# vnminin/phylomap

Measured on NVIDIA B200. Metric: sampled branch-site histories/sec (4-state, 10k-tip tree), higher is better.
Workload: dtype f32

## Files before the change

### phylomap_b200/csrc/pm_host.cu

```cuda
#include <cuda_runtime.h>

#include <algorithm>
#include <chrono>
#include <cmath>
#include <cstdarg>
#include <cstdio>
#include <cstdlib>
#include <cstring>
#include <map>
#include <memory>
#include <mutex>
#include <string>
#include <type_traits>
#include <vector>

#include "../../include/phylomap_b200.h"
#include "pm_launch.cuh"
#include "pm_setup_kernels.cuh"
#include "pm_loglik.cuh"
#include "pm_exp.cuh"
#include "pm_nccl.hpp"
#include "pm_rates.hpp"
#include "pm_tree.hpp"

// ... 859 lines not shown
    const int ntr = ntrees;
    if (n < 2 || n > PM_NMAX) fail(PM_ERR_ARG, "number of states must be in 2..%d", PM_NMAX);
    if (!V.multi && ntr != 1) fail(PM_ERR_ARG, "this sampler takes exactly one tree");
    if (ntr < 1) fail(PM_ERR_ARG, "no trees");
    if (N_total < 0) fail(PM_ERR_ARG, "N must be non-negative");
    if (V.hidden && (n < 4 || (n & 1))) fail(PM_ERR_ARG, "hidden-rate samplers need an even number of states >= 4");
    if (V.two_state && n != 2) fail(PM_ERR_ARG, "this sampler is 2-state only");
    if (V.dic && n > PM_DIC_NMAX) fail(PM_ERR_ARG, "the DIC samplers support at most %d states", PM_DIC_NMAX);
    const int need_prior = V.two_state ? 4 : variant == PM_V_KSMT ? 8 : V.hidden ? 6 : 0;
    if (nprior < need_prior || (need_prior && !prior_)) fail(PM_ERR_ARG, "prior needs %d values", need_prior);
    if (need_prior) prior.assign(prior_, prior_ + nprior);
    pid.assign(pid_, pid_ + n);
    exact = opt.mode == PM_MODE_DETERMINISTIC;
    if (exact && opt.precision != PM_F64) fail(PM_ERR_ARG, "deterministic mode computes in FP64");
    if (exact && V.exp) fail(PM_ERR_ARG, "the direct sampler (maketreelistEXP) runs in production arithmetic only");
    if (opt.rng == PM_RNG_TABLE && (!opt.tab_off || !opt.tab_u)) fail(PM_ERR_ARG, "replay table missing");
    if (opt.rng == PM_RNG_TABLE && !exact) fail(PM_ERR_ARG, "the replay table feeds the deterministic mode only");
    if (opt.rng == PM_RNG_TABLE && (opt.site_offset != 0 || opt.allreduce || opt.nccl_world > 1)) fail(PM_ERR_ARG, "replay runs are single-process");
    if (opt.allreduce && !opt.cuda_stream)
      fail(PM_ERR_ARG, "an allreduce callback needs pm_options.cuda_stream: the collective must be ordered on the stream the chain launches on");
    if (opt.allreduce && opt.nccl_world > 1) fail(PM_ERR_ARG, "give either an allreduce callback or an NCCL clique, not both");
    if (opt.nccl_world > 1 && (!opt.nccl_id || opt.nccl_rank < 0 || opt.nccl_rank >= opt.nccl_world)) fail(PM_ERR_ARG, "bad NCCL clique (nccl_id / nccl_rank / nccl_world)");
    NS = (n == 2) ? 2 : (n == 4) ? 4 : 0;
    W = n + n * n + 1 + (V.dic ? 1 : 0);
    WR = W + 1;
    ncols = ncols_of(variant, n);

    if (!(Omega > 0)) fail(PM_ERR_ARG, "Omega must be positive");
    std::vector<pm::host::Schedule> schedules(ntr);
    for (int ti = 0; ti < ntr; ti++) {
      const pm_tree& x = tr[ti];
      if (x.n_tips != tr[0].n_tips || x.n_edges != tr[0].n_edges) fail(PM_ERR_ARG, "all trees must have the same number of tips");
      if (x.n_sites < 1 || x.n_sites != tr[0].n_sites) fail(PM_ERR_ARG, "n_sites must be >= 1 and equal across trees");
      if (x.n_sites >= (1LL << 31)) fail(PM_ERR_ARG, "at most 2^31 - 1 sites per process");
      if (!x.edge || !x.nen || !x.nodelist || !x.maps_off || !x.maps_len) fail(PM_ERR_ARG, "tree %d: missing field", ti);
      if (!x.states && !x.states_u8) fail(PM_ERR_ARG, "tree %d: states missing", ti);
      try {
        pm::host::build_schedule(x.n_tips, x.n_edges, x.edge, x.nen, x.nodelist, x.root, V.redraw_tips, schedules[ti]);
      } catch (const std::string& msg) { fail(PM_ERR_ARG, "tree %d: %s", ti, msg.c_str()); }
      if (x.maps_off[0] != 0) fail(PM_ERR_ARG, "tree %d: maps_off[0] must be 0", ti);
      for (int e = 0; e < x.n_edges; e++) {
        const long long a = x.maps_off[e], b = x.maps_off[e + 1];
        if (b <= a) fail(PM_ERR_ARG, "tree %d: branch %d has no segments", ti, e + 1);
        if (b - a > 65535) fail(PM_ERR_ARG, "tree %d: branch %d has more than 65535 segments", ti, e + 1);
        for (long long p = a; p < b; p++) {
          if (!(x.maps_len[p] >= 0)) fail(PM_ERR_ARG, "tree %d: negative or NA segment length", ti);
          if (x.maps_state && (x.maps_state[p] < 1 || x.maps_state[p] > n)) fail(PM_ERR_ARG, "tree %d: mapnames out of range", ti);
        }
      }
    }
    return schedules;
  }

  int open_device() {
    int ndev = 0;
    if (cudaGetDeviceCount(&ndev) != cudaSuccess || ndev <= 0) fail(PM_ERR_CUDA, "no CUDA device (there is no CPU fallback)");
    if (opt.device < 0 || opt.device >= ndev) fail(PM_ERR_CUDA, "device %d not present", opt.device);
    CK(cudaSetDevice(opt.device));
    int major = 0, minor = 0, sms = 0;
    CK(cudaDeviceGetAttribute(&major, cudaDevAttrComputeCapabilityMajor, opt.device));
    CK(cudaDeviceGetAttribute(&minor, cudaDevAttrComputeCapabilityMinor, opt.device));
    CK(cudaDeviceGetAttribute(&sms, cudaDevAttrMultiProcessorCount, opt.device));
    if (major != 10) fail(PM_ERR_CUDA, "device %d is sm_%d%d; this library is built for sm_100a only", opt.device, major, minor);
    if (opt.cuda_stream) stream = (cudaStream_t)opt.cuda_stream;
    else { CK(cudaStreamCreateWithFlags(&stream, cudaStreamNonBlocking)); own_stream = true; }
    return sms;
  }

  std::unique_ptr<TreeDev<Real>> create_tree(const pm_tree& x, int ti, pm::host::Schedule&& sch, int sms, cudaStream_t aux,
                                             double& tmax, PhaseTrace& trace) {
    std::unique_ptr<TreeDev<Real>> tp(new TreeDev<Real>());
    TreeDev<Real>& t = *tp;
    t.sch = std::move(sch);
    t.S = x.n_sites;
    t.TS = (t.S + 15) / 16 * 16;
    const int E = x.n_edges, T = x.n_tips;
    const long long S = t.S;
    const bool no_paths = V.exp || V.llonly;
    upload_tips(t, x, aux);
    std::vector<long long> moff(x.maps_off, x.maps_off + E + 1);
    std::vector<Real> elen(E);
    for (int e = 0; e < E; e++) {
      double tot = 0;
      for (long long p = moff[e]; p < moff[e + 1]; p++) tot = tot + x.maps_len[p];
      elen[e] = (Real)tot;
      tmax = std::max(tmax, tot);
    }
    std::vector<double> mlen(x.maps_len, x.maps_len + moff[E]);

    const size_t small_smem = with_ns([&](auto ns) { return pm::Sweep<Real, decltype(ns)::value, false>::small_smem(T); });
    const SmallChoice small = choose_small_kernel(!exact && (NS == 2 || NS == 4) && !no_paths && opt.rng != PM_RNG_TABLE, elen,
                                                  Omega, T, S, sms, small_smem, sw);
    t.small_ok = small.ok;
    t.small_two = small.two;
    const bool pooled_ok = !t.small_ok && !exact && !no_paths && sw.rec_pool;
    RecordPlan rp = plan_records(pooled_ok ? 5 : 0, elen, moff, S, Omega, exact, no_paths, opt.path_capacity);
    if (!rp.fits) rp = plan_records(0, elen, moff, S, Omega, exact, no_paths, opt.path_capacity);
    t.rec_shift = rp.rec_shift;
    t.rec_groups = (S + (1LL << t.rec_shift) - 1) >> t.rec_shift;
    t.chunk = rp.chunk;
    t.paths_grid = dim3((unsigned)rp.gx, (unsigned)rp.ny, 1);
    t.nblocks = rp.gx * rp.ny;
    t.small_chunks = (int)rp.ny;
    t.cap_off_h = std::move(rp.cap_off);
    trace.mark("record capacities");

    plan_partials_slots(t, sms);
    upload(t.up_entries, t.sch.up_entries, stream);
    upload(t.up_off, t.sch.up_off, stream);
    if (!exact && (NS == 2 || NS == 4)) {
      CladeCode cc = encode_clade_schedule(t.sch, S, t.TS, (long long)t.pl_sites * n * (long long)sizeof(Real), V.redraw_tips);
      upload(t.cl_entries, cc.e16, stream);
      upload(t.cl_warp_off, cc.cs.warp_off, stream);
      upload(t.cl_top_entries, cc.top, stream);
      upload(t.cl_top_off, cc.cs.top_off, stream);
      upload(t.cd_entries, cc.d16, stream);
      upload(t.cd_warp_off, cc.cs.down_warp_off, stream);
      upload(t.cd_top, cc.cs.down_top, stream);
      upload(t.cd_top_off, cc.cs.down_top_off, stream);
      upload(t.cd_tips, cc.tips, stream);
      t.P.n_cl_top_levels = (int)cc.cs.top_off.size() - 1;
      t.P.n_cd_top_levels = (int)cc.cs.down_top_off.size() - 1;
      t.P.n_cd_tips = (int)cc.tips.size() / 2;
      if (t.small_ok) {
        const SmallOrder so = small_draw_order(t.sch, cc.cs, elen);
        upload(t.small_down, so.down, stream);
        upload(t.small_border, so.border, stream);
        t.small_order_n = (int)so.border.size();
      }
    }
    upload(t.down_entries, t.sch.down_entries, stream);
    upload(t.down_off, t.sch.down_off, stream);
    upload(t.e_parent, t.sch.e_parent, stream);
    upload(t.e_child, t.sch.e_child, stream);
    upload(t.e_len, elen, stream);
    if (V.dic || V.exp) {
      std::vector<double> eld(E);
      for (int e = 0; e < E; e++) eld[e] = x.edge_length ? x.edge_length[e] : (double)elen[e];
      if (x.edge_length) for (int e = 0; e < E; e++) if (!(eld[e] >= 0)) fail(PM_ERR_ARG, "tree %d: negative or NA edge.length", ti);
      upload(t.e_len_d, eld, stream);
      t.TP.alloc((size_t)E * n * n * sizeof(Real));
      t.ll_partial.alloc((size_t)((S + 31) / 32) * sizeof(double));
    }
    trace.mark("clade schedules + uploads");
    alloc_path_state(t, moff, mlen, elen, sms);
    trace.mark("device buffers");
    return tp;
  }

  void upload_tips(TreeDev<Real>& t, const pm_tree& x, cudaStream_t aux) {
    const int T = x.n_tips;
    t.tipcode.alloc((size_t)T * t.TS);
    CK(cudaMemsetAsync(t.tipcode.p, 0, t.tipcode.bytes, aux));
    t.node_state.alloc((size_t)(2 * T - 1) * t.S);
    CK(cudaMemsetAsync(t.node_state.p, 0, t.node_state.bytes, aux));
    const size_t esz = x.states_u8 ? 1 : 4;
    long long rows_per = std::max<long long>(32, (256LL << 20) / ((long long)T * (long long)esz));
    rows_per = std::min<long long>(rows_per, std::min<long long>(t.S, 32LL * 65535));
    t.tip_stage.alloc((size_t)rows_per * T * esz);
    for (long long s0 = 0; s0 < t.S; s0 += rows_per) {
      const int ns = (int)std::min<long long>(rows_per, t.S - s0);
      const void* src = x.states_u8 ? (const void*)(x.states_u8 + s0 * T) : (const void*)(x.states + s0 * T);
      CK(cudaMemcpyAsync(t.tip_stage.p, src, (size_t)ns * T * esz, cudaMemcpyHostToDevice, aux));
      dim3 g((T + 31) / 32, (ns + 31) / 32), b(32, 8);
      if (x.states_u8)
        pm::k_init_tips<uint8_t><<<g, b, 0, aux>>>(t.tip_stage.template as<uint8_t>(), ns, s0, t.S, t.TS, T, n, V.parity_tips,
                                                     t.tipcode.template as<uint8_t>(), t.node_state.template as<uint8_t>(), err_flag.as<unsigned>());
      else
        pm::k_init_tips<int32_t><<<g, b, 0, aux>>>(t.tip_stage.template as<int32_t>(), ns, s0, t.S, t.TS, T, n, V.parity_tips,
                                                     t.tipcode.template as<uint8_t>(), t.node_state.template as<uint8_t>(), err_flag.as<unsigned>());
    }
    CK(cudaGetLastError());
  }

  void plan_partials_slots(TreeDev<Real>& t, int sms) {
    t.pl_slots = 0;
    t.pl_sites = t.S;
    if (exact || !(NS == 2 || NS == 4) || V.dic || V.exp || V.llonly || !sw.fused) return;
    const size_t smem_lo = ((size_t)n * n + 3 * n) * sizeof(Real);
    const int per_sm = with_ns([&](auto ns) { return pm::Sweep<Real, decltype(ns)::value, false>::fused_blocks_per_sm(smem_lo); });
    if (per_sm < 1) fail(PM_ERR_CUDA, "cudaOccupancyMaxActiveBlocksPerMultiprocessor failed for the fused prune + node-draw kernel");
    t.slots_per_sm = per_sm;
    t.pl_slots = sm_id_range(opt.device, sms) * per_sm;
    t.pl_sites = 32LL * t.pl_slots;
    if (t.pl_sites >= ((t.S + 31) / 32) * 32) {
      t.pl_slots = (int)((t.S + 31) / 32); t.pl_sites = 32LL * t.pl_slots; t.slots_per_sm = 0;
    } else {
      t.slot_busy.alloc((size_t)t.pl_slots * sizeof(int));
      CK(cudaMemsetAsync(t.slot_busy.p, 0, t.slot_busy.bytes, stream));
    }
  }

  void alloc_path_state(TreeDev<Real>& t, const std::vector<long long>& moff, const std::vector<double>& mlen,
                        const std::vector<Real>& elen, int sms) {
    const int E = t.sch.E, T = t.sch.T;
    const long long S = t.S, R = t.cap_off_h.back();
    const bool no_paths = V.exp || V.llonly;
    upload(t.maps_off, moff, stream);
    upload(t.maps_len, mlen, stream);
    upload(t.cap_off, t.cap_off_h, stream);
    if (!no_paths) t.meta.alloc((size_t)E * S * sizeof(uint32_t));
    t.PL.alloc((size_t)(T - 1) * t.pl_sites * n * sizeof(Real));
    for (int b = 0; b < 2 && !no_paths; b++) {
      t.rec_len[b].alloc((size_t)R * t.rec_groups * sizeof(Real));
      t.rec_st[b].alloc((size_t)R * t.rec_groups);
    }
    if (!exact && !no_paths) {
      const long long Wl = (S + 31) / 32;
      t.hard_ballot.alloc((size_t)E * Wl * sizeof(uint32_t));
      const WorkItems w = build_work_items(elen, Omega, S);
      t.wk_total = w.off.back();
      upload(t.wk_hint, w.hint, stream);
      upload(t.wk_off, w.off, stream);
      upload(t.wk_g, w.g, stream);
      t.wk_item.alloc((size_t)std::max<long long>(t.wk_total, 1) * sizeof(unsigned long long));
      pm::k_build_items<<<(unsigned)((t.wk_total + 255) / 256), 256, 0, stream>>>(t.wk_off.template as<long long>(), t.wk_g.template as<int>(), E, Wl,
                                                                                 t.wk_total, t.wk_item.template as<unsigned long long>());
      t.rec_cursor.alloc((size_t)t.small_chunks * t.rec_groups * sizeof(int));
      t.shape.alloc((size_t)E * S * sizeof(uint16_t));
      t.hard_blocks = (int)std::max<long long>(1, std::min<long long>(sms * 4LL, (t.wk_total + 3) / 4));
    }
    t.dw_rows = t.nblocks + 3 * t.hard_blocks;
    t.dw_partial.alloc((size_t)t.dw_rows * n * sizeof(double));
    CK(cudaMemsetAsync(t.dw_partial.p, 0, t.dw_partial.bytes, stream));
    dev_bytes += t.tipcode.bytes + t.node_state.bytes + t.meta.bytes + t.PL.bytes + 2 * (t.rec_len[0].bytes + t.rec_st[0].bytes) +
                 t.dw_partial.bytes + t.hard_ballot.bytes + t.rec_cursor.bytes + t.shape.bytes + t.wk_item.bytes;
  }

  void alloc_model_and_host_buffers(double tmax) {
    jcap = opt.power_capacity > 0 ? opt.power_capacity : 64;
    if (V.exp) jcap = 302;
    else if (opt.power_capacity <= 0) {
      const double lam = Omega * tmax;
      const double want = lam + 10 * std::sqrt(lam) + 24;
      jcap = (int)std::min(16384.0, std::max(64.0, want));
    }
    if (jcap < 2) jcap = 2;
    model.alloc((model_stride() + (size_t)jcap * n * n) * sizeof(Real));
    CK(cudaMallocHost((void**)&model_h, (model_stride() + (size_t)jcap * n * n) * sizeof(Real)));
    memset(model_h, 0, (model_stride() + (size_t)jcap * n * n) * sizeof(Real));
    CK(cudaMallocHost((void**)&rows_h, (size_t)ntrees * WR * sizeof(double)));
    if (cudaHostGetDevicePointer((void**)&rows_h_dev, rows_h, 0) != cudaSuccess) { rows_h_dev = nullptr; (void)cudaGetLastError(); }
    if (opt.nccl_world > 1) nccl = clique(opt.nccl_id, opt.nccl_world, opt.nccl_rank);
    CK(cudaMallocHost((void**)&err_h, sizeof(unsigned)));
    CK(cudaMallocHost((void**)&ctl_h, 2 * sizeof(uint32_t)));
    ctl.alloc(2 * sizeof(uint32_t));
    phase_ns.alloc(2 * sizeof(unsigned long long));
    CK(cudaMemsetAsync(phase_ns.p, 0, phase_ns.bytes, stream));
    if (V.dic) { CK(cudaMallocHost((void**)&q_h, (size_t)n * n * sizeof(double))); q_dev.alloc((size_t)n * n * sizeof(double)); }
    cnt.alloc((size_t)n * n * sizeof(unsigned long long));
    root_out.alloc(sizeof(int));
    CK(cudaMemsetAsync(cnt.p, 0, cnt.bytes, stream));
    CK(cudaMemsetAsync(root_out.p, 0, root_out.bytes, stream));
  }

  int replay_slots_per_iter() const { return (2 * trees[0]->sch.T - 1) + 2 * trees[0]->sch.E; }
  void upload_replay_table() {
    const long long nslots = (long long)ntrees * trees[0]->S * N_total * replay_slots_per_iter();
    std::vector<long long> off(nslots + 1);
    for (long long i = 0; i <= nslots; i++) off[i] = opt.tab_off[i];
    std::vector<double> u(opt.tab_u, opt.tab_u + off[nslots]);
    upload(tab_off, off, stream);
    upload(tab_u, u, stream);
    if (opt.host_tab) replay.reset(new pm::host::ReplaySource(opt.host_tab, opt.host_tab_n));
  }

  void fill_params(TreeDev<Real>& t, int ti) {
    pm::ChainParams<Real>& P = t.P;
    const int T = t.sch.T, E = t.sch.E, spi = replay_slots_per_iter();
    P.n = n; P.T = T; P.E = E; P.S = t.S;
    P.cap_off = t.cap_off.template as<int>();
    P.hard_ballot = t.hard_ballot.template as<uint32_t>(); P.W = (int)((t.S + 31) / 32);
    P.wk_off = t.wk_off.template as<long long>(); P.wk_g = t.wk_g.template as<int>(); P.wk_total = t.wk_total;
    P.wk_hint = t.wk_hint.template as<int>(); P.wk_item = t.wk_item.template as<unsigned long long>();
    P.rec_cursor = t.rec_cursor.template as<int>(); P.chunk = t.chunk; P.easy_blocks = t.nblocks;
    P.shape = t.shape.template as<uint16_t>();
    P.model = model.as<Real>(); P.ppow = model.as<Real>() + model_stride(); P.jcap = jcap;
    P.up_entries = t.up_entries.template as<int>(); P.up_off = t.up_off.template as<int>();
    P.n_up_levels = (int)t.sch.up_off.size() - 1;
    P.cl_entries = t.cl_entries.template as<int>(); P.cl_warp_off = t.cl_warp_off.template as<int>();
    P.cl_top_entries = t.cl_top_entries.template as<int>(); P.cl_top_off = t.cl_top_off.template as<int>();
    P.cd_top = t.cd_top.template as<int>(); P.cd_top_off = t.cd_top_off.template as<int>();
    P.cd_entries = t.cd_entries.template as<int>(); P.cd_warp_off = t.cd_warp_off.template as<int>();
    P.cd_tips = t.cd_tips.template as<long long>();
    P.down_entries = t.down_entries.template as<int>(); P.down_off = t.down_off.template as<int>();
    P.n_down_levels = (int)t.sch.down_off.size() - 1;
    P.e_parent = t.e_parent.template as<int>(); P.e_child = t.e_child.template as<int>();
    P.e_len = t.e_len.template as<Real>();
    P.maps_off = t.maps_off.template as<long long>(); P.maps_len = t.maps_len.template as<double>();
    P.root = t.sch.root;
    P.tipcode = t.tipcode.template as<uint8_t>(); P.TS = t.TS; P.node_state = t.node_state.template as<uint8_t>();
    P.meta = t.meta.template as<uint32_t>(); P.PL = t.PL.template as<Real>();
    P.tile_base = 0; P.pl_S = t.pl_sites; P.rec_shift = t.rec_shift; P.rec_groups = t.rec_groups; P.ctl = nullptr;
    for (int b = 0; b < 2; b++) { P.rec_len[b] = t.rec_len[b].template as<Real>(); P.rec_st[b] = t.rec_st[b].template as<uint8_t>(); }
    P.normalize = V.normalize || !exact; P.full_counts = V.full_counts; P.parity_tips = V.parity_tips;
    P.dw_partial = t.dw_partial.template as<double>(); P.cnt = cnt.as<unsigned long long>();
    P.root_out = root_out.as<int>(); P.err_flag = err_flag.as<unsigned>();
    const uint64_t key = opt.seed + (uint64_t)ti * 0x9E3779B97F4A7C15ull;
    P.rng.k0 = (uint32_t)key; P.rng.k1 = (uint32_t)(key >> 32);
    for (int r = 0; r < 10; r++) { P.rng.rk[2 * r] = P.rng.k0 + (uint32_t)r * 0x9E3779B9u; P.rng.rk[2 * r + 1] = P.rng.k1 + (uint32_t)r * 0xBB67AE85u; }
    P.rng.site0 = (uint32_t)opt.site_offset;
    P.rng.tab_off = opt.rng == PM_RNG_TABLE ? (const int64_t*)tab_off.p : nullptr;
    P.rng.tab_u = opt.rng == PM_RNG_TABLE ? tab_u.as<double>() : nullptr;
    P.rng.tab_site_stride = (int64_t)N_total * spi;
    P.rng.tab_base = (int64_t)ti * t.S * N_total * spi;
    P.rng.slots_per_iter = spi; P.rng.n_nodes = 2 * T - 1;
  }

  void reduce_over_ranks(double* buf, int count) {
    if (nccl) {
      auto& api = pm::host::NcclApi::get();
      const int rc = api.AllReduce(buf, buf, (size_t)count, pm::host::NcclApi::kDouble, pm::host::NcclApi::kSum, nccl, stream);
      if (rc != 0) fail(PM_ERR_CUDA, "ncclAllReduce failed: %s", api.error(rc).c_str());
    } else if (opt.allreduce) {
      if (opt.allreduce(opt.allreduce_ctx, buf, count) != 0) fail(PM_ERR_CUDA, "allreduce callback failed");
    }
  }
  void check_row_errors(const double* rows_host, int nrows) {
    bool any = false;
    for (int i = 0; i < nrows; i++) any = any || rows_host[(size_t)i * WR + W] != 0.0;
    if (!any) return;
    check_device_errors();
    fail(PM_ERR_CUDA, "another rank reported a device error in this sweep; all ranks stop together");
  }

  void ensure_rows(int count) {
    const int need = std::max(count, 1) * ntrees;
    if (need <= rows_cap) return;
    rows.alloc((size_t)need * WR * sizeof(double));
    rows_cap = need;
  }

  void write_fixed_row(const double* r, double* out, int64_t ld, int i) {
    for (int s = 0; s < n; s++) out[i + (int64_t)s * ld] = r[s];
    for (int a = 0; a < n; a++)
      for (int b = 0; b < n; b++) {
        if (a == b) continue;
        const int col = n + a * (n - 1) + b - (a < b ? 1 : 0);
        out[i + (int64_t)col * ld] = r[n + a * n + b];
      }
  }

  void launch_exp_iteration(TreeDev<Real>& t, uint32_t iter, double* row) {
    const int gx = (int)((t.S + 31) / 32);
    Real* TP = t.TP.template as<Real>();
    double* llp = t.ll_partial.template as<double>();
    const size_t smem_b = (size_t)4 * n * sizeof(double) + ((size_t)n * n + ((n * n) & 1)) * sizeof(unsigned) + (size_t)n * n * sizeof(Real);
    const double* el = t.e_len_d.template as<double>();
    with_ns([&](auto ns) {
      constexpr int NSc = decltype(ns)::value;
      begin_timed(0);
      pm::k_loglik<Real, NSc><<<gx, 256, 0, stream>>>(t.P, TP, llp);
      end_timed();
      begin_timed(1);
      pm::k_exp_nodes<Real, NSc><<<gx, 256, 0, stream>>>(t.P, TP, iter);
      end_timed();
      begin_timed(2);
      pm::k_exp_branches<Real, NSc><<<t.paths_grid, 128, smem_b, stream>>>(t.P, TP, el, (Real)Omega, iter, t.chunk);
      end_timed();
    });
    begin_timed(3);
    pm::k_reduce<<<1, 256, 0, stream>>>(t.dw_partial.template as<double>(), t.dw_rows, n, cnt.as<unsigned long long>(),
                                        root_out.as<int>(), row, 0, err_flag.as<unsigned>(), W);
    end_timed();
    launches += 4;
  }

  void run(int count, double* out, int64_t ld) override {
    if (count < 0 || iters_done + count > N_total) fail(PM_ERR_ARG, "cannot run %d more iterations (%d of %d done)", count, iters_done, N_total);
    if (count == 0) return;
    if (ld < count) fail(PM_ERR_ARG, "leading dimension smaller than the number of rows");
    CK(cudaSetDevice(opt.device));
// ... 653 lines not shown
```

### phylomap_b200/csrc/pm_kernels.cuh

```cuda
#pragma once
#include <type_traits>
#include "pm_device.cuh"

namespace pm {

template <typename Real>
struct ChainParams {
  int n, T, E;
  const int* cap_off;
  long long S;
  const Real* model;
  const Real* ppow;
  int jcap;
  const int* up_entries; const int* up_off; int n_up_levels;
  int* rec_cursor;
  const int* cl_entries; const int* cl_warp_off; const int* cl_top_entries; const int* cl_top_off; int n_cl_top_levels;
  const int* cd_top; const int* cd_top_off; int n_cd_top_levels; const int* cd_entries; const int* cd_warp_off;
  const long long* cd_tips; int n_cd_tips;
  const int* down_entries; const int* down_off; int n_down_levels;
  const int* e_parent; const int* e_child; const Real* e_len;
  const long long* maps_off; const double* maps_len;
  int root;
  const uint8_t* tipcode; long long TS;
  uint8_t* node_state; uint32_t* meta; Real* PL;
// ... 1053 lines not shown
    const Real lam = PN::add(PN::mul(lds_real(a_rate + (unsigned)sizeof(Real) * (unsigned)s0, (Real)0), L0),
                             PN::mul(lds_real(a_rate + (unsigned)sizeof(Real) * (unsigned)cs, (Real)0), L1));
    const bool hard = (m > 2) || lam > (Real)PM_LAMBDA_INV;
    const bool ok = TAIL ? (!hard && site_raw < S) : !hard;
    const int k = poisson_inv<Real>(lam, wA);
    red_shared_inc_if(ok && m == 2 && (full || two), a_cnt + 4u * (unsigned)(ps * n + cs));
    add_dwell(s0, L0, ok);
    add_dwell(cs, L1, ok && two);
    const uint32_t newq = (!two && k == 1) ? pos_rand(wB) : q;
    stg_u32_if(ok, meta_b + row, (newq << 16) + (uint32_t)((two ? 2 : 1) + k));
    stg_u16_if(ok, shape_b + row, (uint16_t)(((uint32_t)cs << 11) + ((uint32_t)s0 << 6) + (two ? 1u : 0u)));
    row += Su;
    const unsigned bal = __ballot_sync(0xffffffffu, TAIL ? (hard && site_raw < S) : hard);
    stg_u32_if(bal_writer != 0, bal_b + rowb, bal);
    rowb += Wu;
  };
  auto run = [&](auto tail_c) {
    const std::true_type T{}; const std::false_type F{};
    int i = 0;
    if (nb > 0 && (e0 & 1)) {
      fetch(0, X);
      body(0, T, T, tail_c, X);
      i = 1;
    }
    if (i < nb) fetch(i, X);
    if (i + 1 < nb) fetch(i + 1, Y);
    while (i + 3 < nb) {
      const int stop = min(nb - 4, i + 62);
      for (; i <= stop; i += 2) {
        const Ahead cx = X, cy = Y;
        fetch(i + 2, X); fetch(i + 3, Y);
        body(i, F, T, tail_c, cx);
        body(i + 1, T, F, tail_c, cy);
      }
      flush_dwell();
    }
    for (; i + 1 < nb; i += 2) {
      const Ahead cx = X, cy = Y;
      if (i + 2 < nb) fetch(i + 2, X);
      if (i + 3 < nb) fetch(i + 3, Y);
      body(i, F, T, tail_c, cx);
      body(i + 1, T, F, tail_c, cy);
    }
    if (i < nb) body(i, F, T, tail_c, X);
    flush_dwell();
  };
  if ((long long)(blockIdx.x + 1) * blockDim.x <= S) run(std::false_type()); else run(std::true_type());
  if (NS > 0) {
    const int lane = threadIdx.x & 31, warp = threadIdx.x >> 5;
#pragma unroll
    for (int j = 0; j < NR; j++) {
      double v = lds_real(a_sum + (unsigned)j * (128u * 8u), 0.0);
#pragma unroll
      for (int o = 16; o > 0; o >>= 1) v += __shfl_down_sync(0xffffffffu, v, o);
      if (lane == 0) s_dw[warp * n + j] = v;
    }
  }
  __syncthreads();
  const long long blk = (long long)blockIdx.y * gridDim.x + blockIdx.x;
  if ((int)threadIdx.x < n) {
    double v;
    if (NS > 0) { v = 0; for (int w = 0; w < (int)(blockDim.x >> 5); w++) v += s_dw[w * n + threadIdx.x]; }
    else v = s_dw[threadIdx.x];
    P.dw_partial[blk * n + threadIdx.x] = v;
  }
  for (int i = threadIdx.x; i < n * n; i += blockDim.x) if (s_cnt[i]) atomicAdd(&P.cnt[i], (unsigned long long)s_cnt[i]);
}

template <typename Real>
__device__ __forceinline__ Real rate_or_zero(Real r) { return rate_ok(r) ? r : (Real)0; }

template <typename Real>
struct RunPieces {
  Real L, x, rate;
  int left;
  bool gaps;
  bool firstB;
  uint32_t wB;
  WordStream ws;
  bool joint, pend, run0;
  Real v, sc;
  __device__ __forceinline__ void begin(const RngDesc& d, uint32_t site, uint32_t it, uint32_t e, int run, Real len, Real r,
                                       uint32_t cnt_word, bool single_run, uint32_t wordB) {
    L = len; x = 0; rate = r; left = 0; gaps = false; firstB = single_run; wB = wordB; joint = false;
    if (!rate_ok(r)) return;
    const Real lam = Pin<Real>::mul(r, len);
    if (lam > (Real)PM_LAMBDA_INV) { gaps = true; ws.open(d, site, it, K_BRGAP, e, (uint32_t)run); }
    else { left = poisson_inv<Real>(lam, cnt_word); ws.open(d, site, it, K_BRPOS, e, (uint32_t)run); }
  }
  __device__ __forceinline__ void begin_joint(const RngDesc& d, uint32_t site, uint32_t it, uint32_t e, Real len0, int K, Real lam0,
                                             Real lamT, Real r0, uint32_t wordB) {
    typedef Pin<Real> PN;
    L = len0; x = 0; left = K; gaps = false; firstB = true; wB = wordB; joint = true; pend = false; run0 = true;
    v = 0; rate = PN::div(lam0, lamT); sc = PN::div(lamT, r0);
    ws.open(d, site, it, K_BRPOS, e, 0u);
  }
  __device__ __forceinline__ void second_run(Real len1, Real lamT, Real r1) { L = len1; x = 0; run0 = false; sc = Pin<Real>::div(lamT, r1); }
  __device__ __forceinline__ Real next(bool& last) {
    typedef Pin<Real> PN;
    if (joint) {
      if (!pend && left > 0) {
        uint32_t w;
        if (firstB) { w = wB; firstB = false; } else w = ws.next();
        v = next_order_stat<Real>(v, (Real)1, left, w);
        left--; pend = true;
      }
      if (pend && (!run0 || v < rate)) {
        const Real t2 = min(PN::mul(run0 ? v : PN::sub(v, rate), sc), L);
        const Real piece = max(PN::sub(t2, x), (Real)0);
        x = max(t2, x); pend = false; last = false;
        return piece;
      }
      last = true;
      return PN::sub(L, x);
    }
    if (gaps) {
      const Real g = PN::div(PN::neglog(PN::u01(ws.next())), rate);
      const Real t2 = PN::add(x, g);
      if (t2 < L) { x = t2; last = false; return g; }
      last = true;
      return PN::sub(L, x);
    }
    if (left > 0) {
      uint32_t w;
      if (firstB) { w = wB; firstB = false; } else w = ws.next();
      const Real t2 = next_order_stat<Real>(x, L, left, w);
      const Real piece = PN::sub(t2, x);
      x = t2; left--; last = false;
      return piece;
    }
    last = true;
    return PN::sub(L, x);
  }
};

template <typename Real>
__device__ __noinline__ int count_gaps(RngDesc d, uint32_t site, uint32_t it, uint32_t e, uint32_t run, Real L, Real rate, Real* first) {
  typedef Pin<Real> PN;
  WordStream g; g.open(d, site, it, K_BRGAP, e, run);
  Real x = 0; int k = 0;
  for (;;) {
    const Real gp = PN::div(PN::neglog(PN::u01(g.next())), rate);
    const Real t2 = PN::add(x, gp);
    if (!(t2 < L) || k > 70000) break;
    x = t2; k++;
    if (k == 1) *first = gp;
  }
  return k;
}

template <typename Real>
struct HardItem { uint32_t site, e, meta, ends, shape; };

template <typename Real, int NS>
struct PathWorker {
  static constexpr int NC = NS > 0 ? NS : PM_NMAX;
  static constexpr int NR = NS > 0 ? NS : 1;
  typedef typename StreamSel<Real, false>::type Stream;
  typedef Pin<Real> PN;
  const ChainParams<Real>& P;
  const uint32_t iter; const int first; const int n; const bool full;
  const Real* const sB; const Real* const sBs; const Real* const sPow; const int npow_s;
  unsigned* const s_cnt; double* const s_dw;
  const Real* const s_rate_old; const Real* const s_rate_new;
  const Real* __restrict__ rd_len; const uint8_t* __restrict__ rd_st;
  Real* __restrict__ wr_len; uint8_t* __restrict__ wr_st;
  double Rsum[NR];
  unsigned errbits;
  __device__ __forceinline__ PathWorker(const ChainParams<Real>& P_, uint32_t iter_, int first_, int n_, const Real* sB_, const Real* sBs_,
                                        const Real* sPow_, int npow_s_, unsigned* s_cnt_, double* s_dw_, const Real* rate_old_,
                                        const Real* rate_new_)
      : P(P_), iter(iter_), first(first_), n(n_), full(P_.full_counts != 0), sB(sB_), sBs(sBs_), sPow(sPow_), npow_s(npow_s_),
        s_cnt(s_cnt_), s_dw(s_dw_), s_rate_old(rate_old_), s_rate_new(rate_new_), rd_len(P_.rec_len[(iter_ & 1u) ^ 1u]),
        rd_st(P_.rec_st[(iter_ & 1u) ^ 1u]), wr_len(P_.rec_len[iter_ & 1u]), wr_st(P_.rec_st[iter_ & 1u]), errbits(0) {
#pragma unroll
    for (int j = 0; j < NR; j++) Rsum[j] = 0;
  }
  __device__ __forceinline__ void add_dwell(int s, Real L) {
    if (NS > 0) {
#pragma unroll
      for (int j = 0; j < NR; j++) Rsum[j] += (s == j) ? (double)L : 0.0;
    } else atomicAdd(&s_dw[s], (double)L);
  }

  __device__ __forceinline__ void short_item(const HardItem<Real> it, uint32_t& meta_out, uint16_t& shape_out) {
    const long long site = it.site;
    const int eb = (int)it.e;
    const uint32_t mt = it.meta;
    const int m = (int)(mt & 0xffffu);
    const int nj = (int)(it.shape & 0x3fu);
    const int so0 = (int)((it.shape >> 6) & 0x1fu), so1 = (int)((it.shape >> 11) & 0x1fu);
    const int ps = (int)(it.ends & 0xffu), cs = (int)(it.ends >> 8);
    const Real Le = __ldg(P.e_len + eb);
    const uint32_t gsite = P.rng.site0 + (uint32_t)site;
    uint32_t po_old[4], po_new[4];
    pair_block(P.rng, (uint32_t)site, iter, (uint32_t)eb, po_new);
    if (nj < 2) pair_block(P.rng, (uint32_t)site, iter - 1u, (uint32_t)eb, po_old);
    const uint32_t nA = (eb & 1) ? po_new[2] : po_new[0], nB = (eb & 1) ? po_new[3] : po_new[1];
    Real J0, J1, J2;
    if (nj >= 2) {
      const int ck = eb / P.chunk;
      const int cap0 = __ldg(P.cap_off + ck), cap_c = __ldg(P.cap_off + ck + 1) - cap0;
      const long long sl = ((long long)cap0 * P.rec_groups) + (site >> P.rec_shift) * (long long)cap_c;
      const int rd0 = (int)(mt >> 16);
      J0 = rd_len[sl + min(rd0, cap_c - 1)];
      J1 = PN::add(J0, rd_len[sl + min(rd0 + 1, cap_c - 1)]);
      J2 = m == 4 ? PN::add(J1, rd_len[sl + min(rd0 + 2, cap_c - 1)]) : J1;
    } else {
      const int K = m - 1 - nj;
      const Real p1 = nj == 0 ? Le : pos_dec<Real>(mt >> 16, Le);
      const Real L1r = PN::sub(Le, p1);
      Real qq = (Real)2, sc0 = Le, sc1 = 0;
      if (nj == 1) {
        const Real ro0 = rate_or_zero(s_rate_old[so0]), ro1 = rate_or_zero(s_rate_old[so1]);
        const Real lam0 = PN::mul(ro0, p1), lamT = PN::add(lam0, PN::mul(ro1, L1r));
        qq = PN::div(lam0, lamT); sc0 = PN::div(lamT, ro0); sc1 = PN::div(lamT, ro1);
      }
      const uint32_t oB = (eb & 1) ? po_old[3] : po_old[1];
      uint32_t pw[4] = {0, 0, 0, 0};
      if (K > 1) philox4x32_10(0u, make_slot(K_BRPOS, (uint32_t)eb), iter - 1u, gsite, P.rng.k0, P.rng.k1, pw);
      Real vt0 = 0, vt1 = 0, vt2 = 0;
      int k0o = 0;
      {
        Real v = 0;
#pragma unroll
        for (int j = 0; j < 3; j++) {
          if (j < K) {
            v = next_order_stat<Real>(v, (Real)1, K - j, j == 0 ? oB : pw[j - 1 < 0 ? 0 : j - 1]);
            const bool on0 = v < qq;
            const Real t = on0 ? min(PN::mul(v, sc0), p1) : PN::add(p1, min(PN::mul(PN::sub(v, qq), sc1), L1r));
            k0o += on0 ? 1 : 0;
            if (j == 0) vt0 = t; else if (j == 1) vt1 = t; else vt2 = t;
          }
        }
      }
      J0 = vt0; J1 = vt1; J2 = vt2;
      if (nj == 1) {
        J2 = k0o == 2 ? p1 : vt1;
        J1 = k0o == 0 ? vt0 : k0o == 1 ? p1 : vt1;
        J0 = k0o == 0 ? p1 : vt0;
      }
    }
    auto piece_len = [&](int jx) -> Real {
      const Real hi = jx == 0 ? J0 : jx == 1 ? J1 : (jx == 2 && m == 4) ? J2 : Le;
      const Real lo = jx == 0 ? (Real)0 : jx == 1 ? J0 : jx == 2 ? J1 : J2;
      return PN::sub(hi, lo);
    };
    int nout = 0, S0 = 0, S1 = 0, S2 = 0, S3 = 0;
    Real L0 = 0, L1 = 0, L2 = 0, L3 = 0;
    auto emit = [&](Real L, int sst) {
      const int r = nout;
      if (r == 0) { L0 = L; S0 = sst; } else if (r == 1) { L1 = L; S1 = sst; } else if (r == 2) { L2 = L; S2 = sst; } else { L3 = L; S3 = sst; }
      if (r >= 2) add_dwell(sst, L);
      nout++;
    };
    Stream gst; gst.open(P.rng, (uint32_t)site, iter, K_BRSTATE, (uint32_t)eb, P.err_flag);
    int cur_state = ps, prev = ps;
    Real cur_len = piece_len(0);
#pragma unroll
    for (int pp = 1; pp < 4; pp++) {
      if (pp < m) {
        int st;
        if (pp == m - 1) st = cs;
        else {
          const int jd = m - pp - 1;
          Real wv[NC];
          const Real* M = (jd < npow_s) ? (sPow + jd * n * n) : (P.ppow + (size_t)jd * n * n);
#pragma unroll
          for (int q = 0; q < n; q++) wv[q] = sB[prev * n + q] * M[q * n + cs];
          st = categorical<Real, NC, false>(wv, n, gst.next(), P.err_flag);
        }
        const Real len = piece_len(pp);
        if (full) atomicAdd(&s_cnt[prev * n + st], 1u);
        if (st == cur_state) cur_len = cur_len + len;
        else {
          emit(cur_len, cur_state);
          if (!full) atomicAdd(&s_cnt[cur_state * n + st], 1u);
          cur_state = st; cur_len = len;
        }
        prev = st;
      }
    }
    emit(nout == 0 ? Le : nout == 1 ? PN::sub(Le, L0) : cur_len, cur_state);
    int newm = nout;
    uint32_t newq = 0;
    const Real rn0 = rate_or_zero(s_rate_new[S0]);
    if (nout == 1) {
      add_dwell(S0, L0);
      const int k0n = poisson_inv<Real>(PN::mul(rn0, L0), nA);
      newm += k0n;
      newq = pos_rand(nB);
    } else {
      const Real rn1 = rate_or_zero(s_rate_new[S1]);
      if (nout == 2) {
        newq = pos_enc<Real>(L0, Le);
        L0 = pos_dec<Real>(newq, Le); L1 = PN::sub(Le, L0);
      }
      add_dwell(S0, L0); add_dwell(S1, L1);
      const Real lam0 = PN::mul(rn0, L0), lam1 = PN::mul(rn1, L1);
      if (nout == 2) newm += poisson_inv<Real>(PN::add(lam0, lam1), nA);
      else {
        uint32_t cw[4];
        philox4x32_10(0u, make_slot(K_BRCNT, (uint32_t)eb), iter, gsite, P.rng.k0, P.rng.k1, cw);
        newm += poisson_inv<Real>(lam0, nA) + poisson_inv<Real>(lam1, nB) +
                poisson_inv<Real>(PN::mul(rate_or_zero(s_rate_new[S2]), L2), cw[0]);
        if (nout == 4) newm += poisson_inv<Real>(PN::mul(rate_or_zero(s_rate_new[S3]), L3), cw[1]);
// ... 71 lines not shown
          const Real L1o = PN::sub(Le, p1);
          const Real jlam0 = PN::mul(jr0, p1), jlamT = PN::add(jlam0, PN::mul(jr1, L1o));
          if (r == 0) rp.begin_joint(P.rng, (uint32_t)site, iter - 1u, (uint32_t)eb, p1, poisson_inv<Real>(jlamT, oA), jlam0, jlamT, jr0, oB);
          else rp.second_run(L1o, jlamT, jr1);
          return;
        }
        if (nj == 0) { len = Le; st = (int)((it.shape >> 6) & 0x1fu); }
        else if (nj == 1) { len = r == 0 ? p1 : PN::sub(Le, p1); st = (int)((it.shape >> (r == 0 ? 6 : 11)) & 0x1fu); }
        else { const int q = min(rd0 + r, cap_c - 1); len = rd_len[sbase + q]; st = rd_st[sbase + q]; }
        const uint32_t cw = r == 0 ? oA : r == 1 ? oB : cnt_old.next();
        rp.begin(P.rng, (uint32_t)site, iter - 1u, (uint32_t)eb, r, len, s_rate_old[st], cw, nj == 0, oB);
      };
      if (!first) open_run(0);
      auto next_piece = [&]() -> Real {
        if (first) return (Real)P.maps_len[cp++];
        if (jrun >= nrun) { errbits |= PM_DE_INCONSISTENT; return (Real)0; }
        bool last;
        const Real piece = rp.next(last);
        if (last) { jrun++; if (jrun < nrun) open_run(jrun); }
        return piece;
      };
      nout = 0;
      auto draw_run = [&](int r, Real L, Real rate, uint32_t cw) -> int {
        if (!(rate > (Real)0)) return 0;
        const Real lam = PN::mul(rate, L);
        if (!(lam > (Real)PM_LAMBDA_INV)) return poisson_inv<Real>(lam, cw);
        Real g1 = 0;
        const int k = count_gaps<Real>(P.rng, (uint32_t)site, iter, (uint32_t)eb, (uint32_t)r, L, rate, &g1);
        if (r == 0) { gaps0 = true; gap0 = g1; }
        return k;
      };
      auto emit = [&](Real L, int s) {
        const int r = nout;
        if (replay) {
          wr_len[sbase + wbase + 1 + r] = L; wr_st[sbase + wbase + 1 + r] = (uint8_t)s;
          nout++;
          return;
        }
        if (r == 0) { L0 = L; S0 = s; }
        else if (r == 1) { L1 = L; S1 = s; }
        else if (r < PM_LOCAL_PATH_MAX) { bufL[r] = L; bufS[r] = (uint8_t)s; }
        if (r >= 2) add_dwell(s, L);
        newm += 1;
        if (r >= 2) newm += draw_run(r, L, rate_or_zero(s_rate_new[s]), cnt_new.next());
        nout++;
      };

      int cur_state = (m == 1) ? cs : ps;
      Real cur_len = next_piece();
      int prev = cur_state;
      for (int p = 1; p < m; p++) {
        int st;
        if (p == m - 1) st = cs;
        else {
          const int jd = m - p - 1;
          Real wv[NC];
          const Real* M = (jd < npow_s) ? (sPow + jd * n * n) : (jd < P.jcap ? P.ppow + (size_t)jd * n * n : nullptr);
          if (M) {
#pragma unroll
            for (int c = 0; c < n; c++) wv[c] = M[c * n + cs];
          } else {
#pragma unroll
            for (int c = 0; c < n; c++) wv[c] = (Real)(c == cs);
            for (int r = 0; r < jd; r++) matvec<Real, NC, false>(sBs, n, wv);
          }
#pragma unroll
          for (int c = 0; c < n; c++) wv[c] = sB[prev * n + c] * wv[c];
          st = categorical<Real, NC, false>(wv, n, gst.next(), P.err_flag);
        }
        const Real len = next_piece();
        if (full && !replay) atomicAdd(&s_cnt[prev * n + st], 1u);
        if (st == cur_state) cur_len = cur_len + len;
        else {
          emit(cur_len, cur_state);
          if (!full && !replay) atomicAdd(&s_cnt[cur_state * n + st], 1u);
          cur_state = st; cur_len = len;
        }
        prev = st;
      }
      if (!first && (jrun != nrun)) errbits |= PM_DE_INCONSISTENT;
      emit(nout == 0 ? Le : nout == 1 ? PN::sub(Le, L0) : cur_len, cur_state);
      if (replay) {
        if (nout != (int)wr_len[sbase + wbase]) errbits |= PM_DE_INCONSISTENT;
        break;
      }
      {
        if (nout == 2) {
          newq = pos_enc<Real>(L0, Le);
          L0 = pos_dec<Real>(newq, Le); L1 = PN::sub(Le, L0);
        }
        add_dwell(S0, L0);
        if (nout >= 2) add_dwell(S1, L1);
        const Real rn0 = rate_or_zero(s_rate_new[S0]), rn1 = nout >= 2 ? rate_or_zero(s_rate_new[S1]) : (Real)0;
        const bool together = nout == 2 && !(PN::add(PN::mul(rn0, L0), PN::mul(rn1, L1)) > (Real)PM_LAMBDA_INV);
        if (together) newm += poisson_inv<Real>(PN::add(PN::mul(rn0, L0), PN::mul(rn1, L1)), nA);
        else {
#pragma unroll 1
          for (int r = 0; r < min(nout, 2); r++) {
            const int k = draw_run(r, r == 0 ? L0 : L1, r == 0 ? rn0 : rn1, r == 0 ? nA : nB);
            if (r == 0) k0 = k;
            newm += k;
          }
        }
      }
      if (newm > 65535) { errbits |= PM_DE_M_OVERFLOW; newm = 65535; }
      if (nout == 1) {
        newq = (k0 == 1 && gaps0) ? pos_enc<Real>(gap0, Le) : pos_rand(nB);
        break;
      }
      if (nout == 2) break;
      const bool longp = nout >= 64;
      const int need = nout + (longp ? 1 : 0);
      const int base = atomicAdd(cursor, need);
      newq = (uint32_t)min(base, 65535);
      if (base + need > cap_c || base > 65535) { errbits |= PM_DE_PATH_CAP; break; }
      if (longp) { wr_len[sbase + base] = (Real)nout; wr_st[sbase + base] = 0; }
      if (nout > PM_LOCAL_PATH_MAX) {
        wbase = base;
        continue;
      }
      const int o = base + (longp ? 1 : 0);
      wr_len[sbase + o] = L0; wr_st[sbase + o] = (uint8_t)S0;
      wr_len[sbase + o + 1] = L1; wr_st[sbase + o + 1] = (uint8_t)S1;
      for (int r = 2; r < nout; r++) { wr_len[sbase + o + r] = bufL[r]; wr_st[sbase + o + r] = bufS[r]; }
      break;
    }
    meta_out = PM_META(newm, newq);
    shape_out = PM_SHAPE(min(nout - 1, 63), S0, S1);
  }
};

template <typename Real, int NS, int MINB, int WHICH>
__global__ void __launch_bounds__(128, MINB) k_paths_hard(ChainParams<Real> P, uint32_t iter, int first) {
  if (P.ctl) { iter = P.ctl[0]; first = iter == 0u; }
  constexpr int NC = NS > 0 ? NS : PM_NMAX;
  constexpr int NR = NS > 0 ? NS : 1;
  typedef typename StreamSel<Real, false>::type Stream;
  typedef Pin<Real> PN;
  const int n = NS > 0 ? NS : P.n;
  extern __shared__ __align__(16) unsigned char smem_raw[];
  double* s_dw = reinterpret_cast<double*>(smem_raw);
  unsigned* s_cnt = reinterpret_cast<unsigned*>(s_dw + 4 * n);
  Real* sB = reinterpret_cast<Real*>(s_cnt + n * n + ((n * n) & 1));
  Real* sBs = sB + n * n;
  Real* sVec = sBs + n * n;
  Real* sPow = sVec + 5 * n;
  const int npow_s = min(smem_pow_count<NS, false>(), P.jcap);
  for (int i = threadIdx.x; i < n * n; i += blockDim.x) { sB[i] = P.model[i]; sBs[i] = P.model[n * n + i]; s_cnt[i] = 0; }
  for (int i = threadIdx.x; i < 5 * n; i += blockDim.x) sVec[i] = P.model[2 * n * n + i];
  for (int i = threadIdx.x; i < npow_s * n * n; i += blockDim.x) sPow[i] = P.ppow[i];
  for (int i = threadIdx.x; i < 4 * n; i += blockDim.x) s_dw[i] = 0.0;
  __shared__ HardItem<Real> s_q[4][64];
  __shared__ unsigned short s_stage[4][1024];
  __syncthreads();
  const Real* s_rate_old = sVec + 3 * n;
  const Real* s_rate_new = sVec + 4 * n;
  Real rate_max = 0;
  for (int s = 0; s < n; s++) {
    const Real a = s_rate_old[s], b = s_rate_new[s];
    if (rate_ok(a)) rate_max = max(rate_max, a);
    if (rate_ok(b)) rate_max = max(rate_max, b);
  }
  const long long S = P.S;
  const int W = P.W;
  PathWorker<Real, NS> pw(P, iter, first, n, sB, sBs, sPow, npow_s, s_cnt, s_dw, s_rate_old, s_rate_new);
  const int lane = threadIdx.x & 31, warp = threadIdx.x >> 5;
  const unsigned FULL = 0xffffffffu;

  int nq = 0;
  const long long gw = (long long)blockIdx.x * (blockDim.x >> 5) + warp, NW = (long long)gridDim.x * (blockDim.x >> 5);
  long long wi = gw;
  unsigned long long en_next = wi < P.wk_total ? __ldg(P.wk_item + wi) : 0ull;
  int e = 0, base = 0, total = 0, c = 0, inc = 0;
  long long w0 = 0, prow = 0, crow = 0, erow = 0;
  uint32_t bits = 0;
  bool short_ok = false, finishing = false;
  for (;;) {
    const bool room = nq < 32;
    if (room && base >= total && !finishing) {
      if (wi >= P.wk_total) finishing = true;
      else {
        const unsigned long long en = en_next;
        e = (int)(en >> 32);
        w0 = (long long)((en >> 5) & 0x7ffffffull);
        const int nw = (int)(en & 31ull) + 1;
        wi += NW;
        en_next = wi < P.wk_total ? __ldg(P.wk_item + wi) : 0ull;
        bits = lane < nw ? P.hard_ballot[(long long)e * W + w0 + lane] : 0u;
        c = __popc(bits);
        inc = c;
#pragma unroll
        for (int o = 1; o < 32; o <<= 1) { const int v = __shfl_up_sync(FULL, inc, o); if (lane >= o) inc += v; }
        total = __shfl_sync(FULL, inc, 31);
        base = 0;
        if (total == 0) continue;
        __syncwarp();
        {
          int pos = inc - c;
          uint32_t b2 = bits;
          while (b2) { s_stage[warp][pos++] = (unsigned short)(lane * 32 + __ffs((int)b2) - 1); b2 &= b2 - 1u; }
        }
        __syncwarp();
        short_ok = !first && PN::mul(rate_max, __ldg(P.e_len + e)) <= (Real)(PM_LAMBDA_INV - 0.5);
        prow = (long long)__ldg(P.e_parent + e) * S; crow = (long long)__ldg(P.e_child + e) * S; erow = (long long)e * S;
      }
    }
    if (room && !finishing) {
      const int k = base + lane;
      const bool have = k < total;
      HardItem<Real> it;
      it.e = (uint32_t)e;
      it.site = have ? (uint32_t)(w0 * 32 + s_stage[warp][k]) : 0u;
      it.meta = 0u; it.ends = 0u; it.shape = 0u;
      if (have) {
        it.meta = P.meta[erow + it.site];
        const uint32_t a = P.node_state[prow + it.site], b = P.node_state[crow + it.site];
        if (!first) it.shape = P.shape[erow + it.site];
        it.ends = a | (b << 8);
      }
      bool is_short = false;
      if (WHICH == 0 && have && short_ok) {
        const int m = (int)(it.meta & 0xffffu), njq = (int)(it.shape & 0x3fu);
        is_short = (m == 3 || m == 4) && (njq <= 1 || njq == m - 1);
      }
      const bool mine = have && (WHICH == 1 || is_short);
      if (WHICH == 0 && mine) atomicAnd(P.hard_ballot + (long long)e * W + (it.site >> 5), ~(1u << (it.site & 31u)));
      const unsigned bq = __ballot_sync(FULL, mine);
      if (mine) s_q[warp][nq + __popc(bq & ((1u << lane) - 1u))] = it;
      nq += __popc(bq);
      base += 32;
      __syncwarp();
    }
    if (nq >= 32 || (finishing && nq > 0)) {
      const int take = min(nq, 32);
      nq -= take;
      if (lane < take) {
        const HardItem<Real> it = s_q[warp][nq + lane];
        uint32_t mo; uint16_t so;
        if (WHICH == 0) pw.short_item(it, mo, so);
        else pw.general_item(it, mo, so);
        const long long pe = (long long)it.e * S + it.site;
        P.meta[pe] = mo;
        P.shape[pe] = so;
      }
      __syncwarp();
    } else if (finishing) break;
  }
  if (pw.errbits) atomicOr(P.err_flag, pw.errbits);

  if (NS > 0) {
#pragma unroll
    for (int j = 0; j < NR; j++) {
      double v = pw.Rsum[j];
#pragma unroll
      for (int o = 16; o > 0; o >>= 1) v += __shfl_down_sync(0xffffffffu, v, o);
      if (lane == 0) s_dw[warp * n + j] = v;
    }
  }
  __syncthreads();
  if ((int)threadIdx.x < n) {
    double v;
    if (NS > 0) { v = 0; for (int ww = 0; ww < (int)(blockDim.x >> 5); ww++) v += s_dw[ww * n + threadIdx.x]; }
    else v = s_dw[threadIdx.x];
    P.dw_partial[((long long)P.easy_blocks + (WHICH ? 2LL * gridDim.x : 0LL) + blockIdx.x) * n + threadIdx.x] = v;
  }
  for (int i = threadIdx.x; i < n * n; i += blockDim.x) if (s_cnt[i]) atomicAdd(&P.cnt[i], (unsigned long long)s_cnt[i]);
}

}
```

Before: 71.80 billion.

## Software-pipeline hard-item gathers with cp.async double buffering and shared ballot masks

Restructures the hard-path work loop into a two-stage pipeline. Work-item headers (ballot words, parent/child/length) are prefetched two items ahead, and per-site meta/shape/node_state gathers are issued as cp.async into shared staging while the previous batch is classified. Sub-word loads are widened to aligned 4-byte words, which is why two buffer allocations are padded to a multiple of four bytes. The per-site global atomicAnd on hard_ballot is replaced by a shared-memory mask written back once per item. This aims to hide gather latency and cut global atomics, at the cost of more shared memory, more synchronization and more complex control flow.

```diff
diff --git a/phylomap_b200/csrc/pm_host.cu b/phylomap_b200/csrc/pm_host.cu
--- a/phylomap_b200/csrc/pm_host.cu
+++ b/phylomap_b200/csrc/pm_host.cu
@@ -1035,7 +1035,7 @@
     const int T = x.n_tips;
     t.tipcode.alloc((size_t)T * t.TS);
     CK(cudaMemsetAsync(t.tipcode.p, 0, t.tipcode.bytes, aux));
-    t.node_state.alloc((size_t)(2 * T - 1) * t.S);
+    t.node_state.alloc(((size_t)(2 * T - 1) * t.S + 3) & ~(size_t)3);
     CK(cudaMemsetAsync(t.node_state.p, 0, t.node_state.bytes, aux));
     const size_t esz = x.states_u8 ? 1 : 4;
     long long rows_per = std::max<long long>(32, (256LL << 20) / ((long long)T * (long long)esz));
@@ -1100,7 +1100,7 @@
       pm::k_build_items<<<(unsigned)((t.wk_total + 255) / 256), 256, 0, stream>>>(t.wk_off.template as<long long>(), t.wk_g.template as<int>(), E, Wl,
                                                                                  t.wk_total, t.wk_item.template as<unsigned long long>());
       t.rec_cursor.alloc((size_t)t.small_chunks * t.rec_groups * sizeof(int));
-      t.shape.alloc((size_t)E * S * sizeof(uint16_t));
+      t.shape.alloc(((size_t)E * S * sizeof(uint16_t) + 3) & ~(size_t)3);
       t.hard_blocks = (int)std::max<long long>(1, std::min<long long>(sms * 4LL, (t.wk_total + 3) / 4));
     }
     t.dw_rows = t.nblocks + 3 * t.hard_blocks;
diff --git a/phylomap_b200/csrc/pm_kernels.cuh b/phylomap_b200/csrc/pm_kernels.cuh
--- a/phylomap_b200/csrc/pm_kernels.cuh
+++ b/phylomap_b200/csrc/pm_kernels.cuh
@@ -1229,6 +1229,27 @@
 template <typename Real>
 struct HardItem { uint32_t site, e, meta, ends, shape; };
 
+template <typename Real>
+struct HardHead {
+  uint32_t bits[32];
+  unsigned long long en;
+  int parent, child; Real len;
+};
+struct HardStep {
+  uint32_t site[32], meta[32], shape[32], ps[32], cs[32];
+  int e, w0;
+  uint32_t info;
+};
+struct HardCur {
+  long long prow, crow, erow;
+  int e, w0;
+  uint32_t info;
+};
+__device__ __forceinline__ const void* word_of(const void* p) { return reinterpret_cast<const void*>((uintptr_t)p & ~(uintptr_t)3); }
+__device__ __forceinline__ void cp_async8(unsigned dst, const void* gsrc) {
+  asm volatile("cp.async.ca.shared.global [%0], [%1], 8;" ::"r"(dst), "l"(gsrc) : "memory");
+}
+
 template <typename Real, int NS>
 struct PathWorker {
   static constexpr int NC = NS > 0 ? NS : PM_NMAX;
@@ -1606,15 +1627,13 @@
   for (int i = threadIdx.x; i < 4 * n; i += blockDim.x) s_dw[i] = 0.0;
   __shared__ HardItem<Real> s_q[4][64];
   __shared__ unsigned short s_stage[4][1024];
+  __shared__ HardHead<Real> s_head[4][2];
+  __shared__ HardStep s_step[4][2];
+  __shared__ HardCur s_cur[4];
+  __shared__ uint32_t s_keep[4][2][WHICH == 0 ? 32 : 1];
   __syncthreads();
   const Real* s_rate_old = sVec + 3 * n;
   const Real* s_rate_new = sVec + 4 * n;
-  Real rate_max = 0;
-  for (int s = 0; s < n; s++) {
-    const Real a = s_rate_old[s], b = s_rate_new[s];
-    if (rate_ok(a)) rate_max = max(rate_max, a);
-    if (rate_ok(b)) rate_max = max(rate_max, b);
-  }
   const long long S = P.S;
   const int W = P.W;
   PathWorker<Real, NS> pw(P, iter, first, n, sB, sBs, sPow, npow_s, s_cnt, s_dw, s_rate_old, s_rate_new);
@@ -1622,70 +1641,121 @@
   const unsigned FULL = 0xffffffffu;
 
   int nq = 0;
-  const long long gw = (long long)blockIdx.x * (blockDim.x >> 5) + warp, NW = (long long)gridDim.x * (blockDim.x >> 5);
-  long long wi = gw;
-  unsigned long long en_next = wi < P.wk_total ? __ldg(P.wk_item + wi) : 0ull;
-  int e = 0, base = 0, total = 0, c = 0, inc = 0;
-  long long w0 = 0, prow = 0, crow = 0, erow = 0;
-  uint32_t bits = 0;
-  bool short_ok = false, finishing = false;
+  const long long gw = (long long)blockIdx.x * (blockDim.x >> 5) + warp;
+  const int NW = (int)(gridDim.x * (blockDim.x >> 5));
+  auto fetch_head = [&](int h, long long i, unsigned long long en) {
+    if (i >= P.wk_total) return;
+    const int eh = (int)(en >> 32), nw = (int)(en & 31ull) + 1;
+    const long long wb = (long long)eh * W + (long long)((en >> 5) & 0x7ffffffull);
+    if (lane < nw) cp_async4(smem_addr(&s_head[warp][h].bits[lane]), P.hard_ballot + wb + lane);
+    if (lane == 0) { s_head[warp][h].en = en; cp_async4(smem_addr(&s_head[warp][h].parent), P.e_parent + eh); }
+    if (lane == 1) cp_async4(smem_addr(&s_head[warp][h].child), P.e_child + eh);
+    if (lane == 2) {
+      if (sizeof(Real) == 8) cp_async8(smem_addr(&s_head[warp][h].len), P.e_len + eh);
+      else cp_async4(smem_addr(&s_head[warp][h].len), P.e_len + eh);
+    }
+  };
+  long long wl = gw;
+  unsigned long long en_next = wl + 2 * NW < P.wk_total ? __ldg(P.wk_item + wl + 2 * NW) : 0ull;
+  fetch_head(0, wl, wl < P.wk_total ? __ldg(P.wk_item + wl) : 0ull);
+  fetch_head(1, wl + NW, wl + NW < P.wk_total ? __ldg(P.wk_item + wl + NW) : 0ull);
+  unsigned hpend = 3u;
+  int hs = 0, si = 0;
+  int base = 0, total = 0;
+  bool staged = false;
+  if (lane == 0) s_cur[warp].info = 0u;
   for (;;) {
-    const bool room = nq < 32;
-    if (room && base >= total && !finishing) {
-      if (wi >= P.wk_total) finishing = true;
-      else {
-        const unsigned long long en = en_next;
-        e = (int)(en >> 32);
-        w0 = (long long)((en >> 5) & 0x7ffffffull);
-        const int nw = (int)(en & 31ull) + 1;
-        wi += NW;
-        en_next = wi < P.wk_total ? __ldg(P.wk_item + wi) : 0ull;
-        bits = lane < nw ? P.hard_ballot[(long long)e * W + w0 + lane] : 0u;
-        c = __popc(bits);
-        inc = c;
-#pragma unroll
-        for (int o = 1; o < 32; o <<= 1) { const int v = __shfl_up_sync(FULL, inc, o); if (lane >= o) inc += v; }
-        total = __shfl_sync(FULL, inc, 31);
-        base = 0;
-        if (total == 0) continue;
+    hpend = (hpend & 3u) << 2;
+    while (base >= total && wl < P.wk_total) {
+      if (((hpend | hpend >> 2) >> hs) & 1u) { cp_async_commit(); cp_async_wait<0>(); hpend = 0u; }
+      __syncwarp();
+      const unsigned long long en = s_head[warp][hs].en;
+      const int nw = (int)(en & 31ull) + 1;
+      const uint32_t bits = lane < nw ? s_head[warp][hs].bits[lane] : 0u;
+      const int c = __popc(bits);
+      int inc = c;
+#pragma unroll
+      for (int o = 1; o < 32; o <<= 1) { const int v = __shfl_up_sync(FULL, inc, o); if (lane >= o) inc += v; }
+      total = __shfl_sync(FULL, inc, 31);
+      base = 0;
+      if (total > 0) {
+        int pos = inc - c;
+        uint32_t b2 = bits;
+        while (b2) { s_stage[warp][pos++] = (unsigned short)(lane * 32 + __ffs((int)b2) - 1); b2 &= b2 - 1u; }
+        const uint32_t kp = ((s_cur[warp].info >> 13) & 1u) ^ 1u;
+        if (WHICH == 0) s_keep[warp][kp][lane] = bits;
         __syncwarp();
-        {
-          int pos = inc - c;
-          uint32_t b2 = bits;
-          while (b2) { s_stage[warp][pos++] = (unsigned short)(lane * 32 + __ffs((int)b2) - 1); b2 &= b2 - 1u; }
-        }
-        __syncwarp();
-        short_ok = !first && PN::mul(rate_max, __ldg(P.e_len + e)) <= (Real)(PM_LAMBDA_INV - 0.5);
-        prow = (long long)__ldg(P.e_parent + e) * S; crow = (long long)__ldg(P.e_child + e) * S; erow = (long long)e * S;
-      }
-    }
-    if (room && !finishing) {
+        if (lane == 0) {
+          Real rate_max = 0;
+          for (int s = 0; s < n; s++) {
+            const Real a = s_rate_old[s], b = s_rate_new[s];
+            if (rate_ok(a)) rate_max = max(rate_max, a);
+            if (rate_ok(b)) rate_max = max(rate_max, b);
+          }
+          const bool short_ok = !first && PN::mul(rate_max, s_head[warp][hs].len) <= (Real)(PM_LAMBDA_INV - 0.5);
+          HardCur& cu = s_cur[warp];
+          cu.e = (int)(en >> 32); cu.w0 = (int)((en >> 5) & 0x7ffffffull);
+          cu.prow = (long long)s_head[warp][hs].parent * S; cu.crow = (long long)s_head[warp][hs].child * S; cu.erow = (long long)cu.e * S;
+          cu.info = ((uint32_t)(nw - 1) << 6) | ((uint32_t)short_ok << 12) | (kp << 13) | ((uint32_t)(cu.prow & 3) << 14) |
+                    ((uint32_t)(cu.crow & 3) << 16) | ((uint32_t)(cu.erow & 1) << 18);
+        }
+      }
+      __syncwarp();
+      fetch_head(hs, wl + 2 * NW, en_next);
+      hpend |= 1u << hs;
+      en_next = wl + 3 * NW < P.wk_total ? __ldg(P.wk_item + wl + 3 * NW) : 0ull;
+      wl += NW; hs ^= 1;
+    }
+    const bool issued = base < total;
+    if (issued) {
       const int k = base + lane;
-      const bool have = k < total;
+      HardStep& st = s_step[warp][si];
+      const HardCur& cu = s_cur[warp];
+      if (k < total) {
+        const uint32_t site = (uint32_t)cu.w0 * 32u + s_stage[warp][k];
+        st.site[lane] = site;
+        cp_async4(smem_addr(&st.meta[lane]), P.meta + cu.erow + site);
+        if (!first) cp_async4(smem_addr(&st.shape[lane]), word_of(P.shape + cu.erow + site));
+        cp_async4(smem_addr(&st.ps[lane]), word_of(P.node_state + cu.prow + site));
+        cp_async4(smem_addr(&st.cs[lane]), word_of(P.node_state + cu.crow + site));
+      }
+      if (lane == 0) { st.e = cu.e; st.w0 = cu.w0; st.info = cu.info | (uint32_t)min(total - base, 32) | ((uint32_t)(base + 32 >= total) << 11); }
+      base += 32;
+    }
+    cp_async_commit();
+    cp_async_wait<1>();
+    __syncwarp();
+    if (staged) {
+      const HardStep& st = s_step[warp][si ^ 1];
+      const uint32_t inf = st.info;
+      const bool have = lane < (int)(inf & 63u);
       HardItem<Real> it;
-      it.e = (uint32_t)e;
-      it.site = have ? (uint32_t)(w0 * 32 + s_stage[warp][k]) : 0u;
-      it.meta = 0u; it.ends = 0u; it.shape = 0u;
-      if (have) {
-        it.meta = P.meta[erow + it.site];
-        const uint32_t a = P.node_state[prow + it.site], b = P.node_state[crow + it.site];
-        if (!first) it.shape = P.shape[erow + it.site];
-        it.ends = a | (b << 8);
-      }
+      it.e = (uint32_t)st.e;
+      it.site = st.site[lane];
+      it.meta = st.meta[lane];
+      it.shape = first ? 0u : (st.shape[lane] >> (16u * (((inf >> 18) + it.site) & 1u))) & 0xffffu;
+      const uint32_t a = (st.ps[lane] >> (8u * (((inf >> 14) + it.site) & 3u))) & 0xffu;
+      const uint32_t b = (st.cs[lane] >> (8u * (((inf >> 16) + it.site) & 3u))) & 0xffu;
+      it.ends = a | (b << 8);
       bool is_short = false;
-      if (WHICH == 0 && have && short_ok) {
+      if (WHICH == 0 && have && ((inf >> 12) & 1u)) {
         const int m = (int)(it.meta & 0xffffu), njq = (int)(it.shape & 0x3fu);
         is_short = (m == 3 || m == 4) && (njq <= 1 || njq == m - 1);
       }
       const bool mine = have && (WHICH == 1 || is_short);
-      if (WHICH == 0 && mine) atomicAnd(P.hard_ballot + (long long)e * W + (it.site >> 5), ~(1u << (it.site & 31u)));
+      const int kq = WHICH == 0 ? (int)((inf >> 13) & 1u) : 0;
+      if (WHICH == 0 && mine) atomicAnd(&s_keep[warp][kq][(it.site >> 5) - (uint32_t)st.w0], ~(1u << (it.site & 31u)));
       const unsigned bq = __ballot_sync(FULL, mine);
       if (mine) s_q[warp][nq + __popc(bq & ((1u << lane) - 1u))] = it;
       nq += __popc(bq);
-      base += 32;
+      if (WHICH == 0 && ((inf >> 11) & 1u)) {
+        __syncwarp();
+        if (lane <= (int)((inf >> 6) & 31u)) P.hard_ballot[(long long)st.e * W + st.w0 + lane] = s_keep[warp][kq][lane];
+      }
       __syncwarp();
     }
-    if (nq >= 32 || (finishing && nq > 0)) {
+    const bool done = !staged && !issued;
+    if (nq >= 32 || (done && nq > 0)) {
       const int take = min(nq, 32);
       nq -= take;
       if (lane < take) {
@@ -1698,7 +1768,8 @@
         P.shape[pe] = so;
       }
       __syncwarp();
-    } else if (finishing) break;
+    } else if (done) break;
+    staged = issued; si ^= 1;
   }
   if (pw.errbits) atomicOr(P.err_flag, pw.errbits);
 
```

Result: slower. 69.33 billion (median of 6 runs) (-3.4%).
